# barbagroup/fmm-bem-relaxed

Hardware: AMD Instinct MI355X
Metric: FMM matvecs/s (LaplaceBEM sphere N=1e6 p=10) + achieved HBM GB/s on P2P (higher is better)
Workload: dtype f64; 1 GPU; LaplaceSphericalBEM, 2 disjoint UnitSphere(r=9), N=1048576 panels, p=10, k=3, theta=0.5, ncrit=64, all POTENTIAL; target leaves sharded over 1 GPU(s), 1 all-reduce of y per matvec; n_panels=1048576, p=10, ncrit=64, near_nnz=513008056, m2l_pairs=1959503, boxes=68151, leaves=54524, l2l_rule=complete, l2l_reference_omitted=0

## Files before the change

### fmm-bem-relaxed_amd/csrc/device_launch.hpp

```cpp
#pragma once
#include "device_plan.hpp"
#include "shift_lanes.hpp"

namespace fmmbem {

hipError_t launch_near_assemble(const DevicePlan& d, hipStream_t s);
hipError_t launch_gather_x(const DevicePlan& d, const double* x, hipStream_t s);
hipError_t launch_near_spmv(const DevicePlan& d, hipStream_t s);
bool near_f32_ok(int dof, int max_runs, bool stokes_sym);
hipError_t launch_near_to_f32(const DevicePlan& d, hipStream_t s);
hipError_t launch_near_spmv_f32(const DevicePlan& d, hipStream_t s);
struct HybridStreams { hipStream_t recompute = nullptr; hipEvent_t fork = nullptr, join_recompute = nullptr; };
hipError_t launch_near_hybrid(const DevicePlan& d, hipStream_t s, const HybridStreams& hs);
hipError_t launch_kernel_entries(const DevicePlan& d, int m, double* out, hipStream_t s);
hipError_t launch_panel_setup(int64_t n, const uint32_t* perm, const double* v_orig, int nq, const double* pts, double* cx, double* cy,
                              double* cz, double* nx, double* ny, double* nz, double* area, double* quad, double* vert, hipStream_t s);
int rcg_item_rows();
hipError_t launch_rc_pack(const DevicePlan& d, double* rc_src, double* rc_nrm, hipStream_t s);
hipError_t launch_near_row_eval(const DevicePlan& d, int64_t prow, const int* cols, int n, double* out, hipStream_t s);
hipError_t launch_near_diag(const DevicePlan& d, const int* selfcol, double* out, hipStream_t s);
hipError_t launch_near_matfree(const DevicePlan& d, hipStream_t s);
hipError_t launch_mf_side(const DevicePlan& d, int phase, int* side_cnt, const int64_t* side_ptr, int* side_col, const int* side_row,
                          double* side_val, int64_t nside, hipStream_t s);
hipError_t launch_scatter_y(const DevicePlan& d, double* y, hipStream_t s);
hipError_t launch_assemble_slices(const DevicePlan& d, const double* slices, double* y, int world, const int64_t* d_cut, int64_t chunk,
                                  hipStream_t s);
hipError_t launch_p2m(const DevicePlan& d, int p, hipStream_t s);
hipError_t launch_p2m_table(const DevicePlan& d, double2* tab, hipStream_t s);
hipError_t launch_p2m_table_grad(const DevicePlan& d, double2* tab, hipStream_t s);
hipError_t launch_m2m_level(const DevicePlan& d, const ShiftOpDev& op, int p, int first, int count, hipStream_t s);
hipError_t launch_xch_pack(const DevicePlan& d, int p, double2* send, hipStream_t s);
hipError_t launch_xch_unpack(const DevicePlan& d, int p, const double2* recv, hipStream_t s);
hipError_t launch_mh_prep(const DevicePlan& d, int p, hipStream_t s);
hipError_t launch_m2l(const DevicePlan& d, const DevicePlan* d_dev, int p, hipStream_t s);
bool m2l_rot_supported(int p);
bool shift_rot_supported(int p);
hipError_t launch_m2m_rot(const DevicePlan& d, const RotWork& w, int p, hipStream_t s);
hipError_t launch_l2l_rot(const DevicePlan& d, const RotWork& w, int p, hipStream_t s);
hipError_t launch_m2l_rot(const DevicePlan& d, const DevicePlan* d_dev, int p, hipStream_t s);
bool m2l_rot_long_items(int p);
bool shift_lanes_supported(int p);
hipError_t launch_m2m_lanes(const DevicePlan& d, const ShiftLaneWork& w, int p, hipStream_t s);
hipError_t launch_l2l_lanes(const DevicePlan& d, const ShiftLaneWork& w, int p, hipStream_t s);
unsigned rot_nop_orders_m2l();
unsigned rot_nop_orders_m2m();
unsigned rot_nop_orders_l2l();
int l2p_group_leaves(int kernel);
hipError_t launch_m2l_rot_zero(const DevicePlan& d, int p, hipStream_t s);
hipError_t launch_l2l_level(const DevicePlan& d, const ShiftOpDev& op, int p, int first, int count, hipStream_t s);
hipError_t launch_l2p(const DevicePlan& d, int p, double* y, hipStream_t s);
hipError_t launch_near_assemble_stokes(const DevicePlan& d, hipStream_t s);
hipError_t launch_p2m_stokes(const DevicePlan& d, int p, hipStream_t s);
hipError_t launch_l2p_stokes(const DevicePlan& d, int p, double* y, hipStream_t s);

constexpr int kBatchMax = 8;
struct BatchVecs {
  double* xt[kBatchMax];
  double* yt[kBatchMax];
  double2* M[kBatchMax];
  int nv;
  int width;
};
bool batch_near_ok(const DevicePlan& d);
hipError_t launch_near_spmv_multi(const DevicePlan& d, const BatchVecs& b, hipStream_t s);
bool batch_near_sym3_ok(const DevicePlan& d, int width);
hipError_t launch_near_sym3_multi(const DevicePlan& d, const BatchVecs& b, hipStream_t s);
hipError_t launch_p2m_multi(const DevicePlan& d, const BatchVecs& b, int p, hipStream_t s);

int direct_chunk();
int64_t direct_chunks(int64_t n_sources);
hipError_t launch_direct(const DevicePlan& d, int64_t m, const double* tx, const double* ty, const double* tz, int tstride,
                         const uint8_t* tbc, const double* x, double* part, double* y, hipStream_t s);


}
```

### fmm-bem-relaxed_amd/csrc/kernels_far.hip

```cpp
#include "device_launch.hpp"
#define FMMBEM_INLINE __attribute__((always_inline))

#include <mutex>
#include <type_traits>

namespace fmmbem {

namespace {

constexpr int kWave = 64;
constexpr int kPmaxDev = 16, kSmax = kPmaxDev * (kPmaxDev + 1) / 2;
constexpr double kEps = 1e-12;

struct JK { unsigned char j[136], k[136]; };
__constant__ JK kJK;
__constant__ double kRecip[40];
JK make_jk() {
  JK t;
  int i = 0;
  for (int j = 0; j < 16; ++j)
    for (int k = 0; k <= j; ++k, ++i) { t.j[i] = (unsigned char)j; t.k[i] = (unsigned char)k; }
  return t;
}

// ... 718 lines not shown
      dst[idx] = sum;
    }
    __syncthreads();
  }
}

__global__ __launch_bounds__(kWave) void mh_prep_kernel(DevicePlan d, const int P) {
  const int S = P * (P + 1) / 2;
  const int box = d.mh_box[blockIdx.x];
  const int slot = d.act[blockIdx.y];
  const double2* M = d.M + ((size_t)box * d.nslots + slot) * d.s_max;
  double2* Mh = d.Mh + ((size_t)box * d.nslots + slot) * d.s_max;
  for (int idx = threadIdx.x; idx < S; idx += kWave) {
    const int n = kJK.j[idx], m = kJK.k[idx];
    const double2 v = M[idx];
    const double a = d.tabA[n * n + n + m];
    Mh[m * P - m * (m - 1) / 2 + (n - m)] = mul_i_pow(double2{v.x * a, v.y * a}, -m);
  }
}

constexpr int kL2LWaves = FMMBEM_L2L_WAVES;
__global__ __launch_bounds__(kL2LWaves * kWave) void l2l_kernel(DevicePlan d, ShiftOpDev op, const int P, int first, int count) {
  const int slot_i = blockIdx.y, wg = blockIdx.x, nwg = gridDim.x;
  extern __shared__ double2 lds2[];
  const int S = P * (P + 1) / 2, P2 = P * P, SM = d.s_max, W = S + P2 + op.V;
  const int lane = threadIdx.x & (kWave - 1), w = threadIdx.x / kWave;
  double2* Ls = lds2 + (size_t)w * W;
  double2* Y = Ls + S;
  double2* pv = Y + P2;
  const int slot = d.act[slot_i];
  for (int it = wg * kL2LWaves + w; it < count; it += nwg * kL2LWaves) {
    const int child = d.l2l_child[first + it];
    const int parent = d.box_parent[child];
    const double2* src = d.L + ((size_t)parent * d.nslots + slot) * SM;
    const double2* tab = d.down_tab + (size_t)d.down_cls[child] * d.p2_max;
    __builtin_amdgcn_wave_barrier();
    for (int i = lane; i < S; i += kWave) Ls[i] = src[i];
    for (int i = lane; i < P2; i += kWave) Y[i] = tab[i];
    wave_lds_sync();
    shift_pieces(op, Ls, Y, pv, lane);
    wave_lds_sync();
    double2* dst = d.L + ((size_t)child * d.nslots + slot) * SM;
    for (int idx = lane; idx < S; idx += kWave) {
      const double2 add = shift_apply_row(op, pv, S, idx);
      double2 acc = dst[idx];
      acc.x += add.x; acc.y += add.y;
      dst[idx] = acc;
    }
  }
}

template <class SlotOf>
__device__ __forceinline__ void l2p_stage_group(const DevicePlan& d, int l0, int nl, int slots, int S, int lane, double2* Lw, SlotOf slot_of,
                                                int& my_leaf, int& my_box, int& my_nr, int& g, int& first, int& total) {
  my_leaf = 0; my_box = 0; my_nr = 0;
  if (lane < nl) { my_leaf = d.l2p_leaf[l0 + lane]; my_box = d.leaf_box[my_leaf]; my_nr = d.leaf_nrows[my_leaf]; }
  const int per = slots * S, T = nl * per;
  constexpr int U = 8;
  for (int e0 = 0; e0 < T; e0 += U * kWave) {
    double2 v[U];
#pragma unroll
    for (int u = 0; u < U; ++u) {
      const int e = e0 + u * kWave + lane;
      const int ee = e < T ? e : T - 1;
      const int k = ee / per, rem = ee - k * per, a = rem / S, i = rem - a * S;
      const int box = __shfl(my_box, k, kWave);
      v[u] = d.L[((size_t)box * d.nslots + slot_of(a)) * d.s_max + i];
    }
#pragma unroll
    for (int u = 0; u < U; ++u) {
      const int e = e0 + u * kWave + lane;
      if (e < T) Lw[e] = v[u];
    }
  }
  g = -1; first = 0; total = 0;
  for (int k = 0; k < nl; ++k) {
    const int nr = __shfl(my_nr, k, kWave);
    if (lane >= total && lane < total + nr) { g = k; first = total; }
    total += nr;
  }
}

constexpr int kL2PLeaves = 8, kL2PWaves = 4;
constexpr int kL2PLeavesStokes = 4;
constexpr int kL2PUnrollMax = 12;
static bool l2p_generic() { const char* e = std::getenv("FMMBEM_L2P_GENERIC"); return e && std::atoi(e) != 0; }
template <int PT>
__global__ __launch_bounds__(kL2PWaves * kWave) __attribute__((amdgpu_waves_per_eu(4))) void l2p_kernel(DevicePlan d, const int Prt, double* __restrict__ y, const int store) {
  extern __shared__ double2 l2p_lds[];
  const int P = PT > 0 ? PT : Prt;
  const int S = P * (P + 1) / 2, na = d.n_act;
  double* sPref = reinterpret_cast<double*>(l2p_lds);
  double* sC1 = sPref + S;
  double* sC2 = sC1 + S;
  const int lane = threadIdx.x & (kWave - 1), wave = threadIdx.x / kWave, nwaves = blockDim.x / kWave;
  double2* Lw = l2p_lds + (3 * S + 1) / 2 + (size_t)wave * kL2PLeaves * na * S;
  if (wave == 0) fill_step_tables(d, P, lane, sPref, sC1, sC2);
  __syncthreads();
  for (int gi = blockIdx.x * nwaves + wave; gi < d.n_l2p_grp; gi += gridDim.x * nwaves) {
    const int l0 = d.l2p_grp[gi], nl = d.l2p_grp[gi + 1] - l0;
    wave_lds_sync();
    int g, first, total, my_leaf, my_box, my_nr;
    const int act0 = d.act[0], act1 = d.act[1];
    l2p_stage_group(d, l0, nl, na, S, lane, Lw, [&](int a) { return a == 0 ? act0 : act1; }, my_leaf, my_box, my_nr, g, first, total);
    wave_lds_sync();
    if (nl == 1) { g = 0; first = 0; }
    const int leaf = __shfl(my_leaf, g < 0 ? 0 : g, kWave), box = __shfl(my_box, g < 0 ? 0 : g, kWave);
    const int row0 = d.leaf_row0[leaf], nrows = __shfl(my_nr, g < 0 ? 0 : g, kWave);
    const double c0 = d.box_center[3 * box], c1 = d.box_center[3 * box + 1], c2 = d.box_center[3 * box + 2];
    for (int chunk = 0; chunk < total; chunk += kWave) {
      const int r_in_leaf = chunk + lane - first;
      if (g < 0 || r_in_leaf >= nrows) continue;
      const int64_t i = row0 + r_in_leaf;
      const int tb = d.bc[i] ? 1 : 0;
      const double2* Lt = Lw + (size_t)(g * na + (na == 2 ? tb : 0)) * S;
      const Sph s = cart2sph(d.cx[i] - c0, d.cy[i] - c1, d.cz[i] - c2);
      double r = 0;
      double pn = 1, rhom = 1, er = 1, ei = 0, fact = 1;
      auto order = [&](int m, int& step, auto unrolled) FMMBEM_INLINE {
        int tz = 0;
        if constexpr (decltype(unrolled)::value) asm volatile("" : "+v"(tz), "+v"(r));
        const double *tPref = sPref + tz, *tC1 = sC1 + tz, *tC2 = sC2 + tz;
        const double2* Lm = Lt + tz;
        double p = pn, p1 = p, rhon = rhom;
        const double w = m == 0 ? 1.0 : 2.0;
        auto degree = [&](int n) FMMBEM_INLINE {
          const double mag = rhon * p * tPref[step];
          const double2 Lc = Lm[n * (n + 1) / 2 + m];
          r += w * (Lc.x * (mag * er) - Lc.y * (mag * ei));
          const double pcur = p;
          p = tC1[step] * s.ca * pcur - tC2[step] * p1;
          p1 = pcur;
          rhon *= s.rho;
          ++step;
        };
        if constexpr (decltype(unrolled)::value) {
#pragma unroll
          for (int n = m; n < PT; ++n) degree(n);
        } else {
#pragma nounroll
          for (int n = m; n < P; ++n) degree(n);
        }
        pn = -pn * fact * s.sa;
        fact += 2;
        rhom *= s.rho;
        const double nr = er * s.cb - ei * s.sb, ni = er * s.sb + ei * s.cb;
        er = nr; ei = ni;
      };
      int step = 0;
      if constexpr (PT > 0) {
#pragma unroll
        for (int m = 0; m < PT; ++m) order(m, step, std::true_type{});
      } else {
#pragma nounroll
        for (int m = 0; m < P; ++m) order(m, step, std::false_type{});
      }
      y[i] = (store ? 0.0 : y[i]) + (tb ? -r : r);
    }
  }
}

template <bool TRAC, int PT>
__global__ __launch_bounds__(kL2PWaves * kWave) __attribute__((amdgpu_waves_per_eu(PT > 0 ? 2 : 1))) void l2p_stokes_kernel(DevicePlan d, const int Prt, double* __restrict__ y, const int store) {
  constexpr int NE = TRAC ? 7 : 4, SB = TRAC ? 4 : 0;
  extern __shared__ double2 l2p_lds[];
  const int P = PT > 0 ? PT : Prt;
  const int S = P * (P + 1) / 2;
  double* sPref = reinterpret_cast<double*>(l2p_lds);
  double* sC1 = sPref + S;
  double* sC2 = sC1 + S;
  const int lane = threadIdx.x & (kWave - 1), wave = threadIdx.x / kWave, nwaves = blockDim.x / kWave;
  double2* Lw = l2p_lds + (3 * S + 1) / 2 + (size_t)wave * kL2PLeavesStokes * NE * S;
  if (wave == 0) fill_step_tables(d, P, lane, sPref, sC1, sC2);
  __syncthreads();
  for (int gi = blockIdx.x * nwaves + wave; gi < d.n_l2p_grp; gi += gridDim.x * nwaves) {
    const int l0 = d.l2p_grp[gi], nl = d.l2p_grp[gi + 1] - l0;
    wave_lds_sync();
    int g, first, total, my_leaf, my_box, my_nr;
    l2p_stage_group(d, l0, nl, NE, S, lane, Lw, [&](int e) { return SB + e; }, my_leaf, my_box, my_nr, g, first, total);
    wave_lds_sync();
    if (nl == 1) { g = 0; first = 0; }
    const int leaf = __shfl(my_leaf, g < 0 ? 0 : g, kWave), box = __shfl(my_box, g < 0 ? 0 : g, kWave);
    const int row0 = d.leaf_row0[leaf], nrows = __shfl(my_nr, g < 0 ? 0 : g, kWave);
    const double2* Ls = Lw + (size_t)(g < 0 ? 0 : g) * NE * S;
    const double c0 = d.box_center[3 * box], c1 = d.box_center[3 * box + 1], c2 = d.box_center[3 * box + 2];
    for (int chunk = 0; chunk < total; chunk += kWave) {
      const int r_in_leaf = chunk + lane - first;
      if (g < 0 || r_in_leaf >= nrows) continue;
      const int64_t i = row0 + r_in_leaf;
      if ((d.bc[i] != 0) != TRAC) continue;
      const double tx = d.cx[i], ty = d.cy[i], tz = d.cz[i];
      const Sph s = cart2sph(tx - c0, ty - c1, tz - c2);
      double val[3] = {0, 0, 0};
      double g[4][3] = {{0, 0, 0}, {0, 0, 0}, {0, 0, 0}, {0, 0, 0}};
      double pn = 1, rhom = 1, er = 1, ei = 0, fact = 1;
      const double inv_sa = 1.0 / s.sa, inv_rho = 1.0 / s.rho;
      auto order = [&](int m, int& step, auto unrolled) FMMBEM_INLINE {
        double p = pn, p1 = p, rhon = rhom;
        const double w = m == 0 ? 1.0 : 2.0;
        auto degree = [&](int n) FMMBEM_INLINE {
          int tz = 0;
          if constexpr (decltype(unrolled)::value)
            asm volatile("" : "+v"(tz), "+v"(val[0]), "+v"(val[1]), "+v"(val[2]), "+v"(g[0][0]), "+v"(g[0][1]), "+v"(g[0][2]), "+v"(g[1][0]), "+v"(g[1][1]),
                         "+v"(g[1][2]), "+v"(g[2][0]), "+v"(g[2][1]), "+v"(g[2][2]), "+v"(g[3][0]), "+v"(g[3][1]), "+v"(g[3][2]));
          const double *tPref = sPref + tz, *tC1 = sC1 + tz, *tC2 = sC2 + tz;
          const double2* Lm = Ls + tz;
          const double pref = tPref[step];
          const double mag = rhon * p * pref;
          const double yr = mag * er, yi = mag * ei;
          const double pcur = p;
// ... 199 lines not shown
  if (t >= (int64_t)count * per) return;
  const int idx = (int)(t / per), rem = (int)(t - (int64_t)idx * per), a = rem / S, i = rem - a * S;
  double2* m = d.M + ((size_t)boxes[idx] * d.nslots + d.act[a]) * d.s_max + i;
  if (to_buf) buf[t] = *m; else *m = buf[t];
}

hipError_t launch_xch_pack(const DevicePlan& d, int p, double2* send, hipStream_t s) {
  if (d.xsel_send_box) {
    const int64_t n = (int64_t)d.xsel_send_n * d.n_act * (p * (p + 1) / 2);
    if (n > 0) hipLaunchKernelGGL(xch_list_kernel, dim3((unsigned)((n + 255) / 256)), dim3(256), 0, s, d, p, d.xsel_send_box, d.xsel_send_n, send, 1);
    return hipGetLastError();
  }
  const int64_t n = (int64_t)(d.xch_ptr[d.xch_rank + 1] - d.xch_ptr[d.xch_rank]) * d.n_act * (p * (p + 1) / 2);
  if (n <= 0) return hipSuccess;
  hipLaunchKernelGGL(xch_pack_kernel, dim3((unsigned)((n + 255) / 256)), dim3(256), 0, s, d, p, send);
  return hipGetLastError();
}

hipError_t launch_xch_unpack(const DevicePlan& d, int p, const double2* recv, hipStream_t s) {
  if (d.xsel_recv_box) {
    const int64_t n = (int64_t)d.xsel_recv_n * d.n_act * (p * (p + 1) / 2);
    if (n > 0) hipLaunchKernelGGL(xch_list_kernel, dim3((unsigned)((n + 255) / 256)), dim3(256), 0, s, d, p, d.xsel_recv_box, d.xsel_recv_n, const_cast<double2*>(recv), 0);
    return hipGetLastError();
  }
  const int64_t n = (int64_t)d.xch_ptr[d.xch_world] * d.n_act * (p * (p + 1) / 2);
  if (n <= 0) return hipSuccess;
  hipLaunchKernelGGL(xch_unpack_kernel, dim3((unsigned)((n + 255) / 256)), dim3(256), 0, s, d, p, recv);
  return hipGetLastError();
}

hipError_t launch_mh_prep(const DevicePlan& d, int p, hipStream_t s) {
  if (hipError_t e = upload_constants_once(); e != hipSuccess) return e;
  if (d.n_mh <= 0) return hipSuccess;
  if (p < 1 || p > kPmaxDev) return hipErrorInvalidValue;
  hipLaunchKernelGGL(mh_prep_kernel, dim3(d.n_mh, d.n_act), dim3(kWave), 0, s, d, p);
  return hipGetLastError();
}

hipError_t launch_l2l_level(const DevicePlan& d, const ShiftOpDev& op, int p, int first, int count, hipStream_t s) {
  if (hipError_t e = upload_constants_once(); e != hipSuccess) return e;
  if (count <= 0) return hipSuccess;
  if (p < 1 || p > kPmaxDev) return hipErrorInvalidValue;
  {
    const size_t S = (size_t)p * (p + 1) / 2, P2 = (size_t)p * p;
    const size_t lds = kL2LWaves * (S + P2 + op.V) * sizeof(double2);
    const int blocks = (count + kL2LWaves - 1) / kL2LWaves;
    hipLaunchKernelGGL(l2l_kernel, dim3(blocks < 1024 ? blocks : 1024, d.n_act), dim3(kL2LWaves * kWave), lds, s, d, op, p, first, count);
  }
  return hipGetLastError();
}

int l2p_group_leaves(int kernel) { return kernel == 1 ? kL2PLeavesStokes : kL2PLeaves; }

hipError_t launch_l2p(const DevicePlan& d, int p, double* y, hipStream_t s) {
  constexpr bool store = false;
  if (hipError_t e = upload_constants_once(); e != hipSuccess) return e;
  if (d.n_l2p <= 0) return hipSuccess;
  if (p < 1 || p > kPmaxDev) return hipErrorInvalidValue;
  const int S = p * (p + 1) / 2;
  const size_t per_wave = sizeof(double2) * (size_t)kL2PLeaves * d.n_act * S;
  int nw = (int)((48 * 1024) / per_wave);
  nw = nw < 1 ? 1 : nw > kL2PWaves ? kL2PWaves : nw;
  const int nblk = (d.n_l2p_grp + nw - 1) / nw;
  const size_t lds = sizeof(double2) * (size_t)((3 * S + 1) / 2) + nw * per_wave;
  const dim3 grid(nblk < 256 * 8 ? nblk : 256 * 8), block(nw * kWave);
#define L2P_CASE(PP) case PP: hipLaunchKernelGGL(l2p_kernel<PP>, grid, block, lds, s, d, p, y, store ? 1 : 0); break;
  switch (p <= kL2PUnrollMax && !l2p_generic() ? p : 0) {
    L2P_CASE(1) L2P_CASE(2) L2P_CASE(3) L2P_CASE(4) L2P_CASE(5) L2P_CASE(6) L2P_CASE(7) L2P_CASE(8)
    L2P_CASE(9) L2P_CASE(10) L2P_CASE(11) L2P_CASE(12)
    default: hipLaunchKernelGGL(l2p_kernel<0>, grid, block, lds, s, d, p, y, store ? 1 : 0);
  }
#undef L2P_CASE
  return hipGetLastError();
}

}

namespace fmmbem {
hipError_t launch_p2m_stokes(const DevicePlan& d, int p, hipStream_t s) {
  if (hipError_t e = upload_constants_once(); e != hipSuccess) return e;
  if (d.n_p2m <= 0) return hipSuccess;
  if (p < 1 || p > kPmaxDev) return hipErrorInvalidValue;
  const int nb = (d.n_p2m + 3) / 4;
  const int nblk_r = (d.n_p2m + kP2MWaves - 1) / kP2MWaves;
  const dim3 gr(nblk_r < 256 * 8 ? nblk_r : 256 * 8), br(kP2MWaves * kWave);
  if (d.p2m_tab_g) hipLaunchKernelGGL((p2m_apply_kernel<3>), dim3(nb < 256 * 16 ? nb : 256 * 16), dim3(4 * kWave), 0, s, d, p);
  else if (d.stokes_traction_targets)
    for (int e = 0; e < 7; ++e) hipLaunchKernelGGL((p2m_kernel<1>), gr, br, 0, s, d, p, 5 + e, 4 + e);
  if (!d.stokes_velocity_targets) return hipGetLastError();
  if (d.p2m_tab) {
    hipLaunchKernelGGL((p2m_apply_kernel<4>), dim3(nb < 256 * 16 ? nb : 256 * 16), dim3(4 * kWave), 0, s, d, p);
    return hipGetLastError();
  }
  const int nblk = (d.n_p2m + kP2MWaves - 1) / kP2MWaves;
  const dim3 g(nblk < 256 * 8 ? nblk : 256 * 8), b(kP2MWaves * kWave);
  for (int e = 0; e < 4; ++e) hipLaunchKernelGGL((p2m_kernel<0>), g, b, 0, s, d, p, e + 1, e);
  return hipGetLastError();
}

hipError_t launch_l2p_stokes(const DevicePlan& d, int p, double* y, hipStream_t s) {
  constexpr bool store = false;
  if (hipError_t e = upload_constants_once(); e != hipSuccess) return e;
  if (d.n_l2p <= 0) return hipSuccess;
  if (p < 1 || p > kPmaxDev) return hipErrorInvalidValue;
  const int S = p * (p + 1) / 2;
  for (int trac = 0; trac < 2; ++trac) {
    if (!(trac ? d.stokes_traction_targets : d.stokes_velocity_targets)) continue;
    const size_t per_wave = sizeof(double2) * (size_t)kL2PLeavesStokes * (trac ? 7 : 4) * S;
    int nw = (int)((48 * 1024) / per_wave);
    nw = nw < 1 ? 1 : nw > kL2PWaves ? kL2PWaves : nw;
    const int nblk = (d.n_l2p_grp + nw - 1) / nw;
    const size_t lds = sizeof(double2) * (size_t)((3 * S + 1) / 2) + nw * per_wave;
    const dim3 grid(nblk < 256 * 8 ? nblk : 256 * 8), block(nw * kWave);
#define L2PS_CASE(PP) case PP: if (trac) hipLaunchKernelGGL((l2p_stokes_kernel<true, PP>), grid, block, lds, s, d, p, y, store ? 1 : 0); \
                               else hipLaunchKernelGGL((l2p_stokes_kernel<false, PP>), grid, block, lds, s, d, p, y, store ? 1 : 0); break;
    switch (p <= kL2PUnrollMax && !l2p_generic() ? p : 0) {
      L2PS_CASE(1) L2PS_CASE(2) L2PS_CASE(3) L2PS_CASE(4) L2PS_CASE(5) L2PS_CASE(6) L2PS_CASE(7) L2PS_CASE(8)
      L2PS_CASE(9) L2PS_CASE(10) L2PS_CASE(11) L2PS_CASE(12)
      default: L2PS_CASE(0)
    }
#undef L2PS_CASE
  }
  return hipGetLastError();
// ... 3 lines not shown
```

### fmm-bem-relaxed_amd/csrc/plan.hip

```cpp
#include <hip/hip_runtime.h>

#include <algorithm>
#include <chrono>
#include <climits>
#include <cmath>
#include <complex>
#include <cstdio>
#include <cstring>
#include <cstdlib>
#include <future>
#include <map>
#include <memory>
#include <mutex>
#include <thread>
#include <string>
#include <unordered_map>
#include <vector>

#include "../../include/fmmbem.h"
#include "blockinv.hpp"
#include "device_launch.hpp"
#include "host_plan.hpp"
#include "host_tables.hpp"
#include "m2l_layout.hpp"
// ... 110 lines not shown
  HostPlan hp;
  std::vector<void*> allocs;
  int device = 0;
  bool on_device = false;
  uint64_t fingerprint[2] = {0, 0};
  ~PlanShared() {
    if (!on_device) return;
    DeviceGuard guard(device);
    for (void* p : allocs) (void)hipFree(p);
  }
};

struct fmmbem_plan {
  fmmbem_options opts;
  std::shared_ptr<PlanShared> shared;
  HostPlan& hp;
  DevicePlan d;
  bool on_device = false;
  bool has_bc[2] = {false, false};
  std::vector<void*> allocs;
  std::vector<void*>* alloc_list = nullptr;
  int64_t near_total_doubles = 0, sym_total_doubles = 0;
  fmmbem_plan() : shared(std::make_shared<PlanShared>()), hp(shared->hp) { alloc_list = &shared->allocs; }
  explicit fmmbem_plan(std::shared_ptr<PlanShared> sh) : shared(std::move(sh)), hp(shared->hp) { alloc_list = &allocs; }
  std::shared_ptr<struct MultiDevice> multi;
  fmmbem_plan(const fmmbem_plan&) = default;
  std::vector<std::pair<int, int>> m2m_launch, l2l_launch;
  std::vector<std::pair<int, int>> m2m_shared_launch;
  struct ShiftRot { int item_first = 0, n_items = 0, pairs = 0, level_boxes = 0, pair_first = 0, unit_first = 0, n_units = 0; };
  std::vector<ShiftRot> m2m_rot, m2m_shared_rot, l2l_rot;
  const int *up_rsrc = nullptr, *up_rcls = nullptr, *up_rtgt = nullptr, *up_ritem = nullptr;
  const int *dn_rsrc = nullptr, *dn_rcls = nullptr, *dn_rtgt = nullptr, *dn_ritem = nullptr;
  bool shift_lanes = true;
  int shift_lanes_max = -1;
  int lanes_max(int p, bool m2m) const { return shift_lanes_max >= 0 ? shift_lanes_max : !m2m ? 16384 : p == 10 ? 16384 : p == 9 ? 8192 : 2048; }
  const int* up_unit_ptr = nullptr;
  const double *sl_up_class = nullptr, *sl_dn_class = nullptr, *sl_up_rc = nullptr, *sl_up_xc = nullptr, *sl_dn_rc = nullptr, *sl_dn_xc = nullptr;
  const int32_t *sl_up_rs = nullptr, *sl_up_xs = nullptr, *sl_dn_rs = nullptr, *sl_dn_xs = nullptr;
  size_t sl_rot_off[kShiftLanesPmax + 1] = {}, sl_ax_off[kShiftLanesPmax + 1] = {};
  const double *up_rec = nullptr, *dn_rec = nullptr, *up_stream = nullptr, *dn_stream = nullptr;
  int shift_stream_off[12] = {};
  int shift_rot_min = 2048;
  bool shift_rot = true;
  struct GraphEntry { int region, p; const void* buf; int runs; hipGraphExec_t exec; };
  std::vector<GraphEntry> graphs;
  bool use_graphs = false;
  int m2m_pass(int p, bool shared, hipStream_t s);
  int l2l_pass(int p, hipStream_t s);
  const DevicePlan* d_dev = nullptr;
  bool split_upward = false;
  unsigned pending_mask = 0;
  bool pending_near = false;
  bool result_slices = false;
  int64_t* d_cut = nullptr;
  std::vector<ShiftOpDev> up_ops, down_ops;
  int64_t near_bytes = 0;
  int64_t near_side_entries = 0;
  bool hybrid = false;
  std::vector<uint8_t> near_rec_host;
  std::vector<int64_t> near_off_host, sym_off_host;
  int64_t near_recomputed_pairs = 0;
  int64_t near_f32_floats = 0;
  int last_near_f32 = 0;
  HybridStreams hyb;
  int build_side_lists();
  int64_t n_classes = 0;
  double build_host_ms = 0, build_assemble_ms = 0;
  int timing = 0;
  int last_p = 0;
  static constexpr int kStages = 9, kRing = 64;
  std::vector<hipEvent_t> ev;
  unsigned ev_mask[kRing] = {};
  int64_t ev_count = 0;
  double *stage_x = nullptr, *stage_y = nullptr;
  fmmbem::SolverWs* solver_ws = nullptr;
  hipStream_t own_stream = nullptr;
  struct BlockInverse {
    bool built = false;
    BlockInvDev dev;
    int max_m = 0;
    int64_t doubles = 0;
    double* stage = nullptr;
    size_t stage_doubles = 0;
  };
  BlockInverse binv;
  void block_inverse_free() {
    for (void* p : {(void*)binv.dev.val, (void*)binv.dev.off, (void*)binv.dev.bad, (void*)binv.stage}) if (p) (void)hipFree(p);
    binv = BlockInverse{};
  }
  bool targets = false;
  bool zero_target_rows = false;
  const uint8_t* bc_all[2] = {nullptr, nullptr};
  const double2* p2m_tab_slot[2] = {nullptr, nullptr};
  const uint32_t* d_target_point = nullptr;
  double* y_points = nullptr;
  double* stage_y_targets = nullptr;
  int p2m_targets(int p, hipStream_t s);

  template <class T, class A>
  int upload(const std::vector<T, A>& v, const T** out) {
    *out = nullptr;
    void* p = nullptr;
    const size_t bytes = std::max<size_t>(v.size(), 1) * sizeof(T);
    HIP_TRY(hipMalloc(&p, bytes));
    alloc_list->push_back(p);
    if (!v.empty()) HIP_TRY(hipMemcpy(p, v.data(), v.size() * sizeof(T), hipMemcpyHostToDevice));
// ... 371 lines not shown
    TRY(upload(rec, &d.near_rec));
    if (dof == 3) {
      double *rs = nullptr, *rn = nullptr;
      TRY(alloc((size_t)hp.n * 16, &rs, false)); TRY(alloc((size_t)hp.n * 4, &rn, false));
      HIP_TRY(launch_rc_pack(d, rs, rn, own_stream));
      HIP_TRY(hipStreamSynchronize(own_stream));
      d.rc_src = rs; d.rc_nrm = rn;
    }
  }
  near_rec_host = rec;
  near_off_host = near_off;

  mark("near lists + items");
  TRY(upload(hp.box_center, &d.box_center));
  TRY(upload(T.A, &d.tabA)); TRY(upload(T.invA, &d.tabInvA)); TRY(upload(T.pref, &d.tabPref));
  {
    const int smax = kPmax * (kPmax + 1) / 2;
    std::vector<double> st((size_t)kPmax * (smax + 1) * 4, 0.0);
    for (int p = 1; p <= kPmax; ++p) {
      double* o = st.data() + (size_t)(p - 1) * (smax + 1) * 4;
      for (int m = 0; m < p; ++m)
        for (int n = m; n < p; ++n, o += 4) {
          o[0] = T.pref[n * n + n + m];
          o[1] = n == m ? (double)(2 * m + 1) : (double)(2 * n + 1) * (1.0 / (n - m + 1));
          o[2] = n == m ? 0.0 : (double)(n + m) * (1.0 / (n - m + 1));
        }
    }
    TRY(upload(st, &d.tabStep));
  }

  mark("boxes + harmonic tables");
  TRY(to_device_bc_begin(hp.panels.bc.data()));
  }
  if (part == 1) return FMMBEM_OK;
  alloc_list = &shared->allocs;
  std::vector<int> p2m_leaf, l2p_leaf;
  for (int b : hp.p2m_leaves) p2m_leaf.push_back(hp.box_leaf_index[b]);
  for (int b : hp.l2p_leaves) l2p_leaf.push_back(hp.box_leaf_index[b]);
  d.n_p2m = (int)p2m_leaf.size(); d.n_l2p = (int)l2p_leaf.size();
  TRY(upload(p2m_leaf, &d.p2m_leaf)); TRY(upload(l2p_leaf, &d.l2p_leaf));
  {
    std::vector<int> grp(1, 0);
    int rows = 0;
    const int max_leaves = l2p_group_leaves(d.kernel);
    for (size_t i = 0; i < l2p_leaf.size(); ++i) {
      const int nr = hp.box_body_end[hp.leaf_box[l2p_leaf[i]]] - hp.box_body_begin[hp.leaf_box[l2p_leaf[i]]];
      const int in_group = (int)i - grp.back();
      if (in_group > 0 && (rows + nr > 64 || in_group == max_leaves)) { grp.push_back((int)i); rows = 0; }
      rows += nr;
    }
    grp.push_back((int)l2p_leaf.size());
    d.n_l2p_grp = l2p_leaf.empty() ? 0 : (int)grp.size() - 1;
    TRY(upload(grp, &d.l2p_grp));
  }
  TRY(upload(hp.m2m_parents, &d.m2m_parent)); TRY(upload(hp.l2l_children, &d.l2l_child));
  TRY(upload(hp.box_child_begin, &d.box_child_begin)); TRY(upload(hp.box_child_end, &d.box_child_end));
  TRY(upload(hp.box_parent, &d.box_parent));
  for (size_t l = 0; l + 1 < hp.m2m_level_ptr.size(); ++l)
    if (hp.m2m_level_ptr[l + 1] > hp.m2m_level_ptr[l])
      m2m_launch.emplace_back(hp.m2m_level_ptr[l], hp.m2m_level_ptr[l + 1] - hp.m2m_level_ptr[l]);
  for (size_t l = 0; l + 1 < hp.l2l_level_ptr.size(); ++l)
    if (hp.l2l_level_ptr[l + 1] > hp.l2l_level_ptr[l])
      l2l_launch.emplace_back(hp.l2l_level_ptr[l], hp.l2l_level_ptr[l + 1] - hp.l2l_level_ptr[l]);
  for (size_t l = 0; l + 1 < hp.m2m_shared_ptr.size(); ++l)
    if (hp.m2m_shared_ptr[l + 1] > hp.m2m_shared_ptr[l])
      m2m_shared_launch.emplace_back(hp.m2m_shared_ptr[l], hp.m2m_shared_ptr[l + 1] - hp.m2m_shared_ptr[l]);
  split_upward = hp.opt.shard_upward && hp.opt.shard_world > 1;
  d.xch_rank = hp.opt.shard_rank; d.xch_world = split_upward ? hp.opt.shard_world : 0; d.xch_max = 0;
  for (int r = 0; r < 9; ++r) d.xch_ptr[r] = 0;
  if (split_upward) {
    if (hp.opt.shard_world > 8) return fail(FMMBEM_ERR_UNSUPPORTED, "sharded upward pass: at most 8 shards");
    for (int r = 0; r <= hp.opt.shard_world; ++r) d.xch_ptr[r] = hp.xch_ptr[r];
    for (int r = 0; r < hp.opt.shard_world; ++r) d.xch_max = std::max(d.xch_max, hp.xch_ptr[r + 1] - hp.xch_ptr[r]);
  }
  TRY(upload(hp.xch_box, &d.xch_box));
  if (split_upward && hp.opt.shard_upward == 2) {
    TRY(upload(hp.xsel_send_box, &d.xsel_send_box)); TRY(upload(hp.xsel_recv_box, &d.xsel_recv_box));
    d.xsel_send_n = (int)hp.xsel_send_box.size(); d.xsel_recv_n = (int)hp.xsel_recv_box.size();
  }

  mark("far-field lists");
  {
    std::vector<int> up_cls(nb, 0), down_cls(nb, 0);
    std::unordered_map<IVec3, int, IVec3Hash> seen;
    std::vector<cplx> up_tab, down_tab, h;
    std::vector<double> up_rec_h, dn_rec_h;
    for (int b = 1; b < nb; ++b) {
      const int par = hp.box_parent[b];
      const int32_t v[3] = {hp.box_icoord[3 * par] - hp.box_icoord[3 * b], hp.box_icoord[3 * par + 1] - hp.box_icoord[3 * b + 1],
                            hp.box_icoord[3 * par + 2] - hp.box_icoord[3 * b + 2]};
      const IVec3 key = {v[0], v[1], v[2]};
      auto [it, fresh] = seen.try_emplace(key, (int)seen.size());
      if (fresh) {
        double up[3], down[3];
        for (int k = 0; k < 3; ++k) { up[k] = 0.5 * hp.cell[k] * double(v[k]); down[k] = -up[k]; }
        up_rec_h.resize(up_rec_h.size() + 8); dn_rec_h.resize(dn_rec_h.size() + 8);
        rot_record(up, up_rec_h.data() + up_rec_h.size() - 8); rot_record(down, dn_rec_h.data() + dn_rec_h.size() - 8);
        SphHost s = cart2sph_host(up);
        harmonics(T, true, s.rho, s.alpha, -s.beta, pm, h);
        for (int n = 0; n < pm; ++n)
          for (int m = -n; m <= n; ++m) {
            const cplx y = h[(size_t)n * (n + 1) / 2 + std::abs(m)];
            up_tab.push_back(m < 0 ? std::conj(y) : y);
          }
        s = cart2sph_host(down);
        harmonics(T, true, s.rho, s.alpha, s.beta, pm, h);
// ... 443 lines not shown
    if (!ge) { graphs.push_back(GraphEntry{region, p, buf, 0, nullptr}); ge = &graphs.back(); }
    if (++ge->runs == 1) return body(s);
    if (!ge->exec) {
      static std::mutex capture_mu;
      std::lock_guard<std::mutex> capture_lock(capture_mu);
      HIP_TRY(hipStreamBeginCapture(own_stream, hipStreamCaptureModeThreadLocal));
      const int rc = body(own_stream);
      hipGraph_t g = nullptr;
      const hipError_t e = hipStreamEndCapture(own_stream, &g);
      if (rc != FMMBEM_OK) { if (g) (void)hipGraphDestroy(g); return rc; }
      HIP_TRY(e);
      const hipError_t ei = hipGraphInstantiate(&ge->exec, g, nullptr, nullptr, 0);
      (void)hipGraphDestroy(g);
      HIP_TRY(ei);
    }
    HIP_TRY(hipGraphLaunch(ge->exec, s));
    return FMMBEM_OK;
  };
  if (phase < 2) {
    HIP_TRY(begin(0, s));
    if (targets) {
      DevicePlan dg = d;
      dg.n = hp.n_src;
      HIP_TRY(launch_gather_x(dg, d_x, s));
    } else HIP_TRY(launch_gather_x(d, d_x, s));
    HIP_TRY(end(0, s));
  }
  if (phase == 1) {
    TRY(graphed(1, xbuf, [&](hipStream_t s) -> int {
      HIP_TRY(begin(3, s));
      if (d.kernel == FMMBEM_KERNEL_STOKES_BEM) HIP_TRY(launch_p2m_stokes(d, p, s)); else HIP_TRY(launch_p2m(d, p, s));
      HIP_TRY(end(3, s));
      HIP_TRY(begin(4, s));
      TRY(m2m_pass(p, false, s));
      HIP_TRY(launch_xch_pack(d, p, reinterpret_cast<double2*>(xbuf), s));
      HIP_TRY(end(4, s));
      return FMMBEM_OK;
    }));
    pending_mask = mask;
    pending_near = false;
    return FMMBEM_OK;
  }
  const bool near_f32 = d.near_f32 && p <= opts.near_f32_max_p;
  auto near_field = [&](hipStream_t ns) -> int {
    HIP_TRY(begin(1, ns));
    if (targets && zero_target_rows)
      HIP_TRY(hipMemsetAsync(d.yt + hp.n_src, 0, sizeof(double) * (size_t)(hp.n - hp.n_src), ns));
    if (hybrid) HIP_TRY(launch_near_hybrid(d, ns, hyb));
    else if (near_f32) HIP_TRY(launch_near_spmv_f32(d, ns));
    else if (opts.sparse_local) HIP_TRY(launch_near_spmv(d, ns)); else HIP_TRY(launch_near_matfree(d, ns));
    HIP_TRY(end(1, ns));
    return FMMBEM_OK;
  };
  auto deliver = [&](hipStream_t ns) -> int {
    HIP_TRY(begin(2, ns));
    if (result_slices) {
      HIP_TRY(hipMemcpyAsync(d_y, d.yt + d.row_begin * d.dof, sizeof(double) * (size_t)(d.row_end - d.row_begin) * d.dof,
                             hipMemcpyDeviceToDevice, ns));
    } else if (targets) {
      HIP_TRY(launch_scatter_y(d, d_target_point ? y_points : d_y, ns));
      if (d_target_point) {
        const int64_t nt = hp.n_targets;
        hipLaunchKernelGGL(expand_targets_kernel, dim3((unsigned)((nt + 255) / 256)), dim3(256), 0, ns, d_target_point, y_points, d_y, nt);
        HIP_TRY(hipGetLastError());
      }
    } else {
      if (hp.opt.shard_world > 1) HIP_TRY(hipMemsetAsync(d_y, 0, sizeof(double) * (size_t)hp.n * d.dof, ns));
      HIP_TRY(launch_scatter_y(d, d_y, ns));
    }
    HIP_TRY(end(2, ns));
    return FMMBEM_OK;
  };
  if (phase == 3) {
    TRY(near_field(s));
    pending_mask = mask;
    pending_near = true;
    return FMMBEM_OK;
  }
  const bool near_here = !(phase == 2 && pending_near);
  pending_near = false;
  TRY(graphed((phase == 2 ? 2 : 0) + (near_here ? 0 : 4) + (near_only ? 8 : 0), xbuf, [&](hipStream_t s) -> int {
  if (near_here) TRY(near_field(s));
  if (!near_only) {
    if (phase == 0) {
      HIP_TRY(begin(3, s));
      if (targets) TRY(p2m_targets(p, s));
      else if (d.kernel == FMMBEM_KERNEL_STOKES_BEM) HIP_TRY(launch_p2m_stokes(d, p, s)); else HIP_TRY(launch_p2m(d, p, s));
      HIP_TRY(end(3, s));
      HIP_TRY(begin(4, s));
      TRY(m2m_pass(p, false, s));
      HIP_TRY(end(4, s));
    }
    HIP_TRY(begin(5, s));
    if (phase == 2) {
      HIP_TRY(launch_xch_unpack(d, p, reinterpret_cast<const double2*>(xbuf), s));
      TRY(m2m_pass(p, true, s));
    }
    const bool rot = use_rot(p);
    if (!rot) HIP_TRY(launch_mh_prep(d, p, s));
    HIP_TRY(end(5, s));
    HIP_TRY(begin(6, s));
    if (rot) HIP_TRY(launch_m2l_rot(d, d_dev, p, s));
    else HIP_TRY(launch_m2l(d, d_dev, p, s));
    HIP_TRY(end(6, s));
    HIP_TRY(begin(7, s));
    TRY(l2l_pass(p, s));
    HIP_TRY(end(7, s));
    HIP_TRY(begin(8, s));
    if (d.kernel == FMMBEM_KERNEL_STOKES_BEM) HIP_TRY(launch_l2p_stokes(d, p, d.yt, s));
    else HIP_TRY(launch_l2p(d, p, d.yt, s));
    HIP_TRY(end(8, s));
  }
  return FMMBEM_OK;
  }));
  TRY(deliver(s));
  last_p = p;
  last_near_f32 = near_f32 ? 1 : 0;
  if (tm) { ev_mask[ring] = mask; ++ev_count; }
  return FMMBEM_OK;
}

static int batch_nv() {
  static const int nv = [] {
    const char* e = std::getenv("FMMBEM_BATCH_NV");
    const int v = e ? std::atoi(e) : 4;
    return v == 2 || v == 8 ? v : 4;
  }();
  return nv;
}

int fmmbem_plan::batch_width() const {
  const bool one = on_device && !multi && opts.sparse_local && !hybrid && hp.opt.shard_world <= 1 && !split_upward && !result_slices &&
                   !d.near_f32;
  if (!one) return 1;
  if (opts.kernel == FMMBEM_KERNEL_STOKES_BEM)
    return !targets && opts.stokes_batch_width >= 2 && batch_near_sym3_ok(d, opts.stokes_batch_width) ? opts.stokes_batch_width : 1;
  return !batch_near_ok(d) ? 1 : bat.width ? bat.width : batch_nv();
}

int fmmbem_plan::batch_alloc(hipStream_t s) {
  if (bat.width) return FMMBEM_OK;
  const int w = opts.kernel == FMMBEM_KERNEL_STOKES_BEM ? opts.stokes_batch_width : batch_nv();
  const size_t nt = (size_t)hp.n * d.dof, nm = (size_t)hp.nboxes * d.nslots * d.s_max;
  BatchBufs b;
  std::vector<void*> got;
  auto get = [&](size_t bytes, auto** out) -> bool {
    void* q = nullptr;
    if (hipMalloc(&q, std::max<size_t>(bytes, 1)) != hipSuccess) { (void)hipGetLastError(); return false; }
    got.push_back(q);
    *out = static_cast<std::remove_pointer_t<decltype(out)>>(q);
    return true;
  };
  bool ok = true;
  for (int j = 0; j < w && ok; ++j)
    ok = get(nt * sizeof(double), &b.xt[j]) && get(nt * sizeof(double), &b.yt[j]) && get(nm * sizeof(double2), &b.M[j]) &&
         get(sizeof(DevicePlan), &b.dev[j]);
  for (int j = 0; j < w && ok; ++j) {
    ok = hipMemsetAsync(b.xt[j], 0, nt * sizeof(double), s) == hipSuccess && hipMemsetAsync(b.yt[j], 0, nt * sizeof(double), s) == hipSuccess &&
         hipMemsetAsync(b.M[j], 0, nm * sizeof(double2), s) == hipSuccess;
    DevicePlan dj = d;
    dj.xt = b.xt[j]; dj.yt = b.yt[j]; dj.M = b.M[j];
    ok = ok && hipMemcpy(b.dev[j], &dj, sizeof(DevicePlan), hipMemcpyHostToDevice) == hipSuccess;
  }
  if (!ok) {
    (void)hipStreamSynchronize(s);
    for (void* q : got) (void)hipFree(q);
    (void)hipGetLastError();
// ... 22 lines not shown
    const DevicePlan keep;
    const DevicePlan* keep_dev;
    View(fmmbem_plan& q, int j) : pl(q), keep(q.d), keep_dev(q.d_dev) {
      pl.d.xt = pl.bat.xt[j]; pl.d.yt = pl.bat.yt[j]; pl.d.M = pl.bat.M[j]; pl.d_dev = pl.bat.dev[j];
    }
    ~View() { pl.d = keep; pl.d_dev = keep_dev; }
  };
  for (int j0 = 0; j0 < k; j0 += w) {
    const int nv = std::min(w, k - j0);
    bv.nv = nv;
    for (int j = 0; j < nv; ++j) {
      const double* xj = x + (size_t)(j0 + j) * ldx;
      if (host) { HIP_TRY(hipMemcpyAsync(stage_x, xj, bytes_x, hipMemcpyHostToDevice, s)); xj = stage_x; }
      DevicePlan dg = d;
      dg.xt = bat.xt[j];
      if (targets) dg.n = hp.n_src;
      HIP_TRY(launch_gather_x(dg, xj, s));
      if (targets && zero_target_rows)
        HIP_TRY(hipMemsetAsync(bat.yt[j] + hp.n_src, 0, sizeof(double) * (size_t)(hp.n - hp.n_src), s));
    }
    hipEvent_t* set = timing ? &ev[(size_t)(ev_count % kRing) * 2 * kStages] : nullptr;
    if (set) HIP_TRY(hipEventRecord(set[2 * 1], s));
    if (stokes) HIP_TRY(launch_near_sym3_multi(d, bv, s)); else HIP_TRY(launch_near_spmv_multi(d, bv, s));
    if (set) HIP_TRY(hipEventRecord(set[2 * 1 + 1], s));
    if (!stokes) {
      if (set) HIP_TRY(hipEventRecord(set[2 * 3], s));
      if (targets) {
        for (int f = 0; f < 2; ++f) {
          if (!has_bc[f]) continue;
          DevicePlan dp = d;
          dp.bc = bc_all[f];
          dp.n_act = 1; dp.act[0] = f;
          if (d.p2m_tab) dp.p2m_tab = p2m_tab_slot[f];
          HIP_TRY(launch_p2m_multi(dp, bv, p, s));
        }
      } else HIP_TRY(launch_p2m_multi(d, bv, p, s));
      if (set) HIP_TRY(hipEventRecord(set[2 * 3 + 1], s));
    }
    if (set) {
      ev_mask[ev_count % kRing] = stokes ? (1u << 1) : (1u << 1) | (1u << 3);
      ++ev_count;
    }
    for (int j = 0; j < nv; ++j) {
      double* yj = host ? sy : y + (size_t)(j0 + j) * ldy;
      {
        View view(*this, j);
        if (stokes) HIP_TRY(launch_p2m_stokes(d, p, s));
        TRY(m2m_pass(p, false, s));
        const bool rot = use_rot(p);
        if (!rot) HIP_TRY(launch_mh_prep(d, p, s));
        if (rot) HIP_TRY(launch_m2l_rot(d, d_dev, p, s));
        else HIP_TRY(launch_m2l(d, d_dev, p, s));
        TRY(l2l_pass(p, s));
        if (stokes) HIP_TRY(launch_l2p_stokes(d, p, d.yt, s)); else HIP_TRY(launch_l2p(d, p, d.yt, s));
        if (targets) {
          HIP_TRY(launch_scatter_y(d, d_target_point ? y_points : yj, s));
          if (d_target_point) {
            const int64_t nt = hp.n_targets;
            hipLaunchKernelGGL(expand_targets_kernel, dim3((unsigned)((nt + 255) / 256)), dim3(256), 0, s, d_target_point, y_points, yj, nt);
            HIP_TRY(hipGetLastError());
          }
        } else HIP_TRY(launch_scatter_y(d, yj, s));
      }
      if (host) HIP_TRY(hipMemcpyAsync(y + (size_t)(j0 + j) * ldy, sy, bytes_y, hipMemcpyDeviceToHost, s));
    }
  }
  if (host) HIP_TRY(hipStreamSynchronize(s));
  last_p = p;
  return FMMBEM_OK;
}

extern "C" {

void fmmbem_options_default(fmmbem_options* o) {
  if (!o) return;
  std::memset(o, 0, sizeof(*o));
  o->kernel = FMMBEM_KERNEL_LAPLACE_BEM;
  o->p_max = 10;
  o->quad_k = 3;
  o->theta = 0.5;
  o->ncrit = 64;
  o->sparse_local = 1;
  o->shard_world = 1;
  o->quad_k_fine = 25;
  o->mu = 1e-3;
  o->near_stream_fraction = 1.0;
  o->near_f32_max_p = 0;
  o->stokes_batch_width = 0;
}

static void fingerprint_vertices(const double* v, size_t n_panels, uint64_t out[2]) {
  const size_t words = n_panels * 9;
  const int nt = words < (1u << 20) ? 1 : (int)std::min<unsigned>(16, std::max(1u, std::thread::hardware_concurrency()));
  std::vector<uint64_t> part((size_t)nt * 2);
  auto work = [&](int t) {
    const size_t w0 = words * t / nt, w1 = words * (t + 1) / nt;
    uint64_t a = 0x9E3779B97F4A7C15ull + t, b = 0xC2B2AE3D27D4EB4Full ^ (uint64_t)t;
    for (size_t i = w0; i < w1; ++i) {
      uint64_t x;
      std::memcpy(&x, v + i, 8);
      a = (a ^ x) * 0x100000001B3ull; a ^= a >> 29;
      b += x * 0xFF51AFD7ED558CCDull; b = (b << 27) | (b >> 37); b *= 0xC4CEB9FE1A85EC53ull;
    }
    part[2 * t] = a; part[2 * t + 1] = b;
  };
  if (nt == 1) work(0);
  else {
    host_parallel(nt, [&](int t) { work(t); });
// ... 1285 lines not shown
```

Before: 615.3 matvecs/s.

## Fold scatter_y into L2P and simplify L2P recurrence with prescaled coefficients

L2P now writes its result straight to the permuted user output when every row is covered by an L2P leaf, so the separate scatter_y pass is skipped for Laplace BEM single-shard runs. The staged local coefficients are prescaled by the prefactor table in LDS, and the Legendre/rho recurrence is merged into one scaled term using compile-time coefficients for unrolled orders. This removes one full-vector read/write pass and some per-term multiplies. In exchange, the stores become scattered writes through perm, and when graphs are used the L2P launch moves outside the captured graph as an extra launch.

```diff
diff --git a/fmm-bem-relaxed_amd/csrc/device_launch.hpp b/fmm-bem-relaxed_amd/csrc/device_launch.hpp
--- a/fmm-bem-relaxed_amd/csrc/device_launch.hpp
+++ b/fmm-bem-relaxed_amd/csrc/device_launch.hpp
@@ -48,7 +48,7 @@
 int l2p_group_leaves(int kernel);
 hipError_t launch_m2l_rot_zero(const DevicePlan& d, int p, hipStream_t s);
 hipError_t launch_l2l_level(const DevicePlan& d, const ShiftOpDev& op, int p, int first, int count, hipStream_t s);
-hipError_t launch_l2p(const DevicePlan& d, int p, double* y, hipStream_t s);
+hipError_t launch_l2p(const DevicePlan& d, int p, double* y, hipStream_t s, const uint32_t* perm = nullptr, double* y_out = nullptr);
 hipError_t launch_near_assemble_stokes(const DevicePlan& d, hipStream_t s);
 hipError_t launch_p2m_stokes(const DevicePlan& d, int p, hipStream_t s);
 hipError_t launch_l2p_stokes(const DevicePlan& d, int p, double* y, hipStream_t s);
diff --git a/fmm-bem-relaxed_amd/csrc/kernels_far.hip b/fmm-bem-relaxed_amd/csrc/kernels_far.hip
--- a/fmm-bem-relaxed_amd/csrc/kernels_far.hip
+++ b/fmm-bem-relaxed_amd/csrc/kernels_far.hip
@@ -794,13 +794,15 @@
 
 template <class SlotOf>
 __device__ __forceinline__ void l2p_stage_group(const DevicePlan& d, int l0, int nl, int slots, int S, int lane, double2* Lw, SlotOf slot_of,
-                                                int& my_leaf, int& my_box, int& my_nr, int& g, int& first, int& total) {
+                                                int& my_leaf, int& my_box, int& my_nr, int& g, int& first, int& total,
+                                                const double* scale = nullptr) {
   my_leaf = 0; my_box = 0; my_nr = 0;
   if (lane < nl) { my_leaf = d.l2p_leaf[l0 + lane]; my_box = d.leaf_box[my_leaf]; my_nr = d.leaf_nrows[my_leaf]; }
   const int per = slots * S, T = nl * per;
   constexpr int U = 8;
   for (int e0 = 0; e0 < T; e0 += U * kWave) {
     double2 v[U];
+    double sc[U];
 #pragma unroll
     for (int u = 0; u < U; ++u) {
       const int e = e0 + u * kWave + lane;
@@ -808,10 +810,12 @@
       const int k = ee / per, rem = ee - k * per, a = rem / S, i = rem - a * S;
       const int box = __shfl(my_box, k, kWave);
       v[u] = d.L[((size_t)box * d.nslots + slot_of(a)) * d.s_max + i];
+      sc[u] = scale ? scale[i] : 1.0;
     }
 #pragma unroll
     for (int u = 0; u < U; ++u) {
       const int e = e0 + u * kWave + lane;
+      if (scale) { v[u].x *= sc[u]; v[u].y *= sc[u]; }
       if (e < T) Lw[e] = v[u];
     }
   }
@@ -827,24 +831,38 @@
 constexpr int kL2PLeavesStokes = 4;
 constexpr int kL2PUnrollMax = 12;
 static bool l2p_generic() { const char* e = std::getenv("FMMBEM_L2P_GENERIC"); return e && std::atoi(e) != 0; }
+__host__ __device__ constexpr double l2p_c1(int n, int m) { return n == m ? (double)(2 * m + 1) : (double)(2 * n + 1) * (1.0 / (double)(n - m + 1)); }
+__host__ __device__ constexpr double l2p_c2(int n, int m) { return n == m ? 0.0 : (double)(n + m) * (1.0 / (double)(n - m + 1)); }
+__device__ inline void fill_l2p_tables(const DevicePlan& d, int P, int S, int lane, bool steps, double* sG, double* sC1, double* sC2) {
+  for (int i = lane; i < S; i += kWave) {
+    const int n = kJK.j[i], m = kJK.k[i];
+    sG[i] = (m == 0 ? 1.0 : 2.0) * d.tabPref[n * n + n + m];
+    if (steps) {
+      const int t = m * P - m * (m - 1) / 2 + (n - m);
+      sC1[t] = n == m ? (double)(2 * m + 1) : (double)(2 * n + 1) * kRecip[n - m + 1];
+      sC2[t] = n == m ? 0.0 : (double)(n + m) * kRecip[n - m + 1];
+    }
+  }
+}
 template <int PT>
-__global__ __launch_bounds__(kL2PWaves * kWave) __attribute__((amdgpu_waves_per_eu(4))) void l2p_kernel(DevicePlan d, const int Prt, double* __restrict__ y, const int store) {
+__global__ __launch_bounds__(kL2PWaves * kWave) __attribute__((amdgpu_waves_per_eu(4))) void l2p_kernel(DevicePlan d, const int Prt, double* __restrict__ y, const int store,
+                                                                                                     const uint32_t* __restrict__ perm, double* __restrict__ yout) {
   extern __shared__ double2 l2p_lds[];
   const int P = PT > 0 ? PT : Prt;
   const int S = P * (P + 1) / 2, na = d.n_act;
-  double* sPref = reinterpret_cast<double*>(l2p_lds);
-  double* sC1 = sPref + S;
+  double* sG = reinterpret_cast<double*>(l2p_lds);
+  double* sC1 = sG + S;
   double* sC2 = sC1 + S;
   const int lane = threadIdx.x & (kWave - 1), wave = threadIdx.x / kWave, nwaves = blockDim.x / kWave;
   double2* Lw = l2p_lds + (3 * S + 1) / 2 + (size_t)wave * kL2PLeaves * na * S;
-  if (wave == 0) fill_step_tables(d, P, lane, sPref, sC1, sC2);
+  if (wave == 0) fill_l2p_tables(d, P, S, lane, PT == 0, sG, sC1, sC2);
   __syncthreads();
   for (int gi = blockIdx.x * nwaves + wave; gi < d.n_l2p_grp; gi += gridDim.x * nwaves) {
     const int l0 = d.l2p_grp[gi], nl = d.l2p_grp[gi + 1] - l0;
     wave_lds_sync();
     int g, first, total, my_leaf, my_box, my_nr;
     const int act0 = d.act[0], act1 = d.act[1];
-    l2p_stage_group(d, l0, nl, na, S, lane, Lw, [&](int a) { return a == 0 ? act0 : act1; }, my_leaf, my_box, my_nr, g, first, total);
+    l2p_stage_group(d, l0, nl, na, S, lane, Lw, [&](int a) { return a == 0 ? act0 : act1; }, my_leaf, my_box, my_nr, g, first, total, sG);
     wave_lds_sync();
     if (nl == 1) { g = 0; first = 0; }
     const int leaf = __shfl(my_leaf, g < 0 ? 0 : g, kWave), box = __shfl(my_box, g < 0 ? 0 : g, kWave);
@@ -855,25 +873,28 @@
       if (g < 0 || r_in_leaf >= nrows) continue;
       const int64_t i = row0 + r_in_leaf;
       const int tb = d.bc[i] ? 1 : 0;
+      const int64_t dst = perm ? (int64_t)perm[i] : i;
       const double2* Lt = Lw + (size_t)(g * na + (na == 2 ? tb : 0)) * S;
       const Sph s = cart2sph(d.cx[i] - c0, d.cy[i] - c1, d.cz[i] - c2);
+      const double z = s.rho * s.ca, rho2 = s.rho * s.rho;
       double r = 0;
       double pn = 1, rhom = 1, er = 1, ei = 0, fact = 1;
       auto order = [&](int m, int& step, auto unrolled) FMMBEM_INLINE {
         int tz = 0;
         if constexpr (decltype(unrolled)::value) asm volatile("" : "+v"(tz), "+v"(r));
-        const double *tPref = sPref + tz, *tC1 = sC1 + tz, *tC2 = sC2 + tz;
         const double2* Lm = Lt + tz;
-        double p = pn, p1 = p, rhon = rhom;
-        const double w = m == 0 ? 1.0 : 2.0;
+        double q = pn * rhom, q1 = q;
         auto degree = [&](int n) FMMBEM_INLINE {
-          const double mag = rhon * p * tPref[step];
           const double2 Lc = Lm[n * (n + 1) / 2 + m];
-          r += w * (Lc.x * (mag * er) - Lc.y * (mag * ei));
-          const double pcur = p;
-          p = tC1[step] * s.ca * pcur - tC2[step] * p1;
-          p1 = pcur;
-          rhon *= s.rho;
+          const double u = fma(Lc.x, er, -(Lc.y * ei));
+          r = fma(u, q, r);
+          double k1, k2;
+          if constexpr (decltype(unrolled)::value) { k1 = l2p_c1(n, m); k2 = l2p_c2(n, m); }
+          else { k1 = sC1[step]; k2 = sC2[step]; }
+          const double zq = z * q;
+          const double qn = n == m ? k1 * zq : fma(k1, zq, -(k2 * (rho2 * q1)));
+          q1 = q;
+          q = qn;
           ++step;
         };
         if constexpr (decltype(unrolled)::value) {
@@ -897,7 +918,8 @@
 #pragma nounroll
         for (int m = 0; m < P; ++m) order(m, step, std::false_type{});
       }
-      y[i] = (store ? 0.0 : y[i]) + (tb ? -r : r);
+      const double v = (store ? 0.0 : y[i]) + (tb ? -r : r);
+      if (perm) yout[dst] = v; else y[i] = v;
     }
   }
 }
@@ -1203,11 +1225,11 @@
 
 int l2p_group_leaves(int kernel) { return kernel == 1 ? kL2PLeavesStokes : kL2PLeaves; }
 
-hipError_t launch_l2p(const DevicePlan& d, int p, double* y, hipStream_t s) {
+hipError_t launch_l2p(const DevicePlan& d, int p, double* y, hipStream_t s, const uint32_t* perm, double* y_out) {
   constexpr bool store = false;
   if (hipError_t e = upload_constants_once(); e != hipSuccess) return e;
   if (d.n_l2p <= 0) return hipSuccess;
-  if (p < 1 || p > kPmaxDev) return hipErrorInvalidValue;
+  if (p < 1 || p > kPmaxDev || (perm && !y_out)) return hipErrorInvalidValue;
   const int S = p * (p + 1) / 2;
   const size_t per_wave = sizeof(double2) * (size_t)kL2PLeaves * d.n_act * S;
   int nw = (int)((48 * 1024) / per_wave);
@@ -1215,11 +1237,11 @@
   const int nblk = (d.n_l2p_grp + nw - 1) / nw;
   const size_t lds = sizeof(double2) * (size_t)((3 * S + 1) / 2) + nw * per_wave;
   const dim3 grid(nblk < 256 * 8 ? nblk : 256 * 8), block(nw * kWave);
-#define L2P_CASE(PP) case PP: hipLaunchKernelGGL(l2p_kernel<PP>, grid, block, lds, s, d, p, y, store ? 1 : 0); break;
+#define L2P_CASE(PP) case PP: hipLaunchKernelGGL(l2p_kernel<PP>, grid, block, lds, s, d, p, y, store ? 1 : 0, perm, y_out); break;
   switch (p <= kL2PUnrollMax && !l2p_generic() ? p : 0) {
     L2P_CASE(1) L2P_CASE(2) L2P_CASE(3) L2P_CASE(4) L2P_CASE(5) L2P_CASE(6) L2P_CASE(7) L2P_CASE(8)
     L2P_CASE(9) L2P_CASE(10) L2P_CASE(11) L2P_CASE(12)
-    default: hipLaunchKernelGGL(l2p_kernel<0>, grid, block, lds, s, d, p, y, store ? 1 : 0);
+    default: hipLaunchKernelGGL(l2p_kernel<0>, grid, block, lds, s, d, p, y, store ? 1 : 0, perm, y_out);
   }
 #undef L2P_CASE
   return hipGetLastError();
diff --git a/fmm-bem-relaxed_amd/csrc/plan.hip b/fmm-bem-relaxed_amd/csrc/plan.hip
--- a/fmm-bem-relaxed_amd/csrc/plan.hip
+++ b/fmm-bem-relaxed_amd/csrc/plan.hip
@@ -186,6 +186,12 @@
   unsigned pending_mask = 0;
   bool pending_near = false;
   bool result_slices = false;
+  bool l2p_scatter = false;
+  bool l2p_delivers(bool near_only, int phase) const {
+    if (!l2p_scatter || result_slices || near_only || phase != 0) return false;
+    const char* e = std::getenv("FMMBEM_L2P_SCATTER");
+    return !(e && std::atoi(e) == 0);
+  }
   int64_t* d_cut = nullptr;
   std::vector<ShiftOpDev> up_ops, down_ops;
   int64_t near_bytes = 0;
@@ -663,6 +669,9 @@
     grp.push_back((int)l2p_leaf.size());
     d.n_l2p_grp = l2p_leaf.empty() ? 0 : (int)grp.size() - 1;
     TRY(upload(grp, &d.l2p_grp));
+    int64_t covered = 0;
+    for (int lf : l2p_leaf) covered += hp.box_body_end[hp.leaf_box[lf]] - hp.box_body_begin[hp.leaf_box[lf]];
+    l2p_scatter = d.kernel == FMMBEM_KERNEL_LAPLACE_BEM && !targets && hp.opt.shard_world <= 1 && d.n_l2p > 0 && covered == (int64_t)hp.n;
   }
   TRY(upload(hp.m2m_parents, &d.m2m_parent)); TRY(upload(hp.l2l_children, &d.l2l_child));
   TRY(upload(hp.box_child_begin, &d.box_child_begin)); TRY(upload(hp.box_child_end, &d.box_child_end));
@@ -1212,9 +1221,11 @@
     HIP_TRY(end(1, ns));
     return FMMBEM_OK;
   };
+  const bool fold = l2p_delivers(near_only, phase);
   auto deliver = [&](hipStream_t ns) -> int {
     HIP_TRY(begin(2, ns));
-    if (result_slices) {
+    if (fold) {
+    } else if (result_slices) {
       HIP_TRY(hipMemcpyAsync(d_y, d.yt + d.row_begin * d.dof, sizeof(double) * (size_t)(d.row_end - d.row_begin) * d.dof,
                              hipMemcpyDeviceToDevice, ns));
     } else if (targets) {
@@ -1239,7 +1250,7 @@
   }
   const bool near_here = !(phase == 2 && pending_near);
   pending_near = false;
-  TRY(graphed((phase == 2 ? 2 : 0) + (near_here ? 0 : 4) + (near_only ? 8 : 0), xbuf, [&](hipStream_t s) -> int {
+  TRY(graphed((phase == 2 ? 2 : 0) + (near_here ? 0 : 4) + (near_only ? 8 : 0) + (fold ? 16 : 0), xbuf, [&](hipStream_t s) -> int {
   if (near_here) TRY(near_field(s));
   if (!near_only) {
     if (phase == 0) {
@@ -1268,11 +1279,13 @@
     HIP_TRY(end(7, s));
     HIP_TRY(begin(8, s));
     if (d.kernel == FMMBEM_KERNEL_STOKES_BEM) HIP_TRY(launch_l2p_stokes(d, p, d.yt, s));
-    else HIP_TRY(launch_l2p(d, p, d.yt, s));
+    else if (!fold) HIP_TRY(launch_l2p(d, p, d.yt, s));
+    else if (!graph_ok) HIP_TRY(launch_l2p(d, p, d.yt, s, d.perm, d_y));
     HIP_TRY(end(8, s));
   }
   return FMMBEM_OK;
   }));
+  if (fold && graph_ok) HIP_TRY(launch_l2p(d, p, d.yt, s, d.perm, d_y));
   TRY(deliver(s));
   last_p = p;
   last_near_f32 = near_f32 ? 1 : 0;
@@ -1401,8 +1414,12 @@
         if (rot) HIP_TRY(launch_m2l_rot(d, d_dev, p, s));
         else HIP_TRY(launch_m2l(d, d_dev, p, s));
         TRY(l2l_pass(p, s));
-        if (stokes) HIP_TRY(launch_l2p_stokes(d, p, d.yt, s)); else HIP_TRY(launch_l2p(d, p, d.yt, s));
-        if (targets) {
+        const bool fold = l2p_delivers(false, 0);
+        if (stokes) HIP_TRY(launch_l2p_stokes(d, p, d.yt, s));
+        else if (fold) HIP_TRY(launch_l2p(d, p, d.yt, s, d.perm, yj));
+        else HIP_TRY(launch_l2p(d, p, d.yt, s));
+        if (fold) {
+        } else if (targets) {
           HIP_TRY(launch_scatter_y(d, d_target_point ? y_points : yj, s));
           if (d_target_point) {
             const int64_t nt = hp.n_targets;
```

New measurement: 623.9 matvecs/s (median of 6 runs). +1.4%, better.
